# mountaindust/Parasitoids

Measured on AMD Instinct MI355X. Metric: grid-days/sec on 4096^2 fp64 domain, higher is better.
Workload: dtype f64; 1 GPU; C3 synthetic stack: N=4097 (nominal 4096^2), 30 Gaussian day kernels K=2049, reference torus P=5121, FFT size 5184 (fast mode), prob model, one replica stack per GPU; dom_len=4097, ndays=30, P=5121, fft_len=5184, kernels_direct=False, full_column_pipeline=True

## Files before the change

### include/parasitoid_hip.h

```cpp
#ifndef PARASITOID_HIP_H
#define PARASITOID_HIP_H
#include <stdint.h>

#ifdef __cplusplus
extern "C" {
#endif

#define PS_OK 0
#define PS_ERR_NO_DEVICE (-1)
#define PS_ERR_OOM (-2)
#define PS_ERR_BAD_SHAPE (-3)
#define PS_ERR_BAD_ARG (-4)
#define PS_ERR_UNSUPPORTED (-5)
#define PS_ERR_HIP (-6)
#define PS_ERR_HPROB_BOUNDS (-7)
#define PS_ERR_PMF_NEGATIVE (-8)
#define PS_ERR_FLIGHT_PROB (-9)
#define PS_ERR_STATE (-10)
#define PS_ERR_EMPTY (-11)

#define PS_MODE_EXACT 0
#define PS_MODE_FAST 1
#define PS_MODE_FOLD 2
#define PS_MODE_AUTO 3

typedef struct ps_solver ps_solver;
typedef struct ps_model ps_model;

typedef struct ps_day_stats {
  int64_t nnz;
  double sum;
  double delta;
  double padmax;
  int32_t flag;
  int32_t pad_;
} ps_day_stats;

int ps_version(void);
int ps_device_count(void);
const char* ps_last_error(void);
int ps_device_info(int device, char* name, int n, int* cus, int64_t* hbm_bytes);
int ps_row_live_units(int P, int M, int np, int nd, const int32_t* ranges, int32_t* day, int32_t* unit, int cap);
int ps_row_fwd_info(int fft_len, int* np, int* persistent);
int ps_row_fwd_stage_info(int fft_len, int K, int* staged);
int64_t ps_row_fwd_stage_lds(int fft_len, int K);
int64_t ps_row_fwd_stage_bytes(int np, int K);
int ps_row_fwd_stage_slot(int K, int r, int e, int col);
int ps_row_fwd_stage_walk(int K, int64_t rows, int64_t row, int r, int nstaged, int64_t* image);


int ps_solver_create(ps_solver** out, int device, int dom_len, int max_shape, int mode);
int ps_fast_size(int dom_len, int max_shape);
int ps_solver_retarget(ps_solver* s, int max_shape);
int ps_solver_destroy(ps_solver* s);
int ps_solver_info(ps_solver* s, int* dom_len, int* P, int* Pfft, int* H);
int ps_solver_sync(ps_solver* s);
int ps_solver_set_option(ps_solver* s, const char* key, double value);
int ps_solver_get_option(ps_solver* s, const char* key, double* value);
int ps_solver_kernels_direct(ps_solver* s);
int ps_solver_pipeline(ps_solver* s);
int ps_solver_deferred_info(ps_solver* s, int* pending, int64_t* counts);
int ps_solver_auto_info(ps_solver* s, int* first_fold_day, int* fold_fft);
int ps_solver_auto_route(ps_solver* s, int first, int count, int32_t* owner);

int ps_solver_set_state_coo(ps_solver* s, const int32_t* row, const int32_t* col,
                            const double* val, int64_t nnz);

int ps_solver_fftconv2_coo(ps_solver* s, const int32_t* row, const int32_t* col,
                           const double* val, int64_t nnz, int kshape);

int ps_solver_get_cursol(ps_solver* s, double negval, double stat_scale, int renorm,
                         ps_day_stats* stats);

int ps_solver_back_solve(ps_solver* s, int nfilt, const int64_t* off, const int32_t* row,
                         const int32_t* col, const double* val, double negval,
// ... 450 lines not shown
```

### parasitoids_amd/_lib.py

```python
import ctypes as C
import os

import numpy as np

_HERE = os.path.dirname(os.path.abspath(__file__))
LIB_PATH = os.path.join(_HERE, 'libparasitoid_hip.so')

PS_OK = 0
PS_ERR_NO_DEVICE = -1
PS_ERR_OOM = -2
PS_ERR_BAD_SHAPE = -3
PS_ERR_BAD_ARG = -4
PS_ERR_UNSUPPORTED = -5
PS_ERR_HIP = -6
PS_ERR_HPROB_BOUNDS = -7
PS_ERR_PMF_NEGATIVE = -8
PS_ERR_FLIGHT_PROB = -9
PS_ERR_STATE = -10
PS_ERR_EMPTY = -11

MODE_EXACT = 0
MODE_FAST = 1
MODE_FOLD = 2
MODE_AUTO = 3

REC_CHAIN, REC_BACK, REC_STATE, REC_WSUM = 0, 1, 2, 3
REC_NONE = -1


class DayStats(C.Structure):
    _fields_ = [('nnz', C.c_int64), ('sum', C.c_double), ('delta', C.c_double),
                ('padmax', C.c_double), ('flag', C.c_int32), ('pad_', C.c_int32)]


class HipError(RuntimeError):
    def __init__(self, code, msg):
        super().__init__('libparasitoid_hip error %d: %s' % (code, msg))
        self.code = code


_I32P = C.POINTER(C.c_int32)
_I64P = C.POINTER(C.c_int64)
_F64P = C.POINTER(C.c_double)
_VP = C.c_void_p

SIGNATURES = {
    'ps_version': (C.c_int, []),
    'ps_device_count': (C.c_int, []),
    'ps_last_error': (C.c_char_p, []),
    'ps_device_info': (C.c_int, [C.c_int, C.c_char_p, C.c_int, _I32P, _I64P]),
    'ps_row_live_units': (C.c_int, [C.c_int, C.c_int, C.c_int, C.c_int, _I32P, _I32P, _I32P, C.c_int]),
    'ps_row_fwd_info': (C.c_int, [C.c_int, _I32P, _I32P]),
    'ps_row_fwd_stage_info': (C.c_int, [C.c_int, C.c_int, _I32P]),
    'ps_row_fwd_stage_lds': (C.c_int64, [C.c_int, C.c_int]),
    'ps_row_fwd_stage_bytes': (C.c_int64, [C.c_int, C.c_int]),
    'ps_row_fwd_stage_slot': (C.c_int, [C.c_int, C.c_int, C.c_int, C.c_int]),
    'ps_row_fwd_stage_walk': (C.c_int, [C.c_int, C.c_int64, C.c_int64, C.c_int, C.c_int, _I64P]),
    'ps_solver_create': (C.c_int, [C.POINTER(_VP), C.c_int, C.c_int, C.c_int, C.c_int]),
    'ps_solver_destroy': (C.c_int, [_VP]),
    'ps_solver_info': (C.c_int, [_VP, _I32P, _I32P, _I32P, _I32P]),
    'ps_solver_sync': (C.c_int, [_VP]),
    'ps_solver_set_option': (C.c_int, [_VP, C.c_char_p, C.c_double]),
    'ps_solver_get_option': (C.c_int, [_VP, C.c_char_p, _F64P]),
    'ps_solver_set_state_coo': (C.c_int, [_VP, _I32P, _I32P, _F64P, C.c_int64]),
    'ps_solver_fftconv2_coo': (C.c_int, [_VP, _I32P, _I32P, _F64P, C.c_int64, C.c_int]),
    'ps_solver_get_cursol': (C.c_int, [_VP, C.c_double, C.c_double, C.c_int, C.POINTER(DayStats)]),
    'ps_solver_back_solve': (C.c_int, [_VP, C.c_int, _I64P, _I32P, _I32P, _F64P, C.c_double,
                                       C.c_double, C.POINTER(DayStats)]),
    'ps_chain_set_kernels': (C.c_int, [_VP, C.c_int, _I64P, _I32P, _I32P, _I32P, _F64P]),
    'ps_chain_run': (C.c_int, [_VP, C.c_int, C.c_int, C.c_double, C.c_double, C.c_int]),
    'ps_chain_stats': (C.c_int, [_VP, C.c_int, C.c_int, C.POINTER(DayStats)]),
    'ps_chain_run_release': (C.c_int, [_VP, C.c_int, C.c_int, C.c_double, C.c_int, C.c_int, _F64P,
                                       C.POINTER(C.c_int)]),
    'ps_record_stats': (C.c_int, [_VP, C.c_int, C.c_int, C.c_double, C.c_double, C.c_int,
                                  C.POINTER(DayStats)]),
    'ps_solver_retarget': (C.c_int, [_VP, C.c_int]),
    'ps_fast_size': (C.c_int, [C.c_int, C.c_int]),
    'ps_solver_kernels_direct': (C.c_int, [_VP]),
    'ps_solver_pipeline': (C.c_int, [_VP]),
    'ps_solver_deferred_info': (C.c_int, [_VP, _I32P, _I64P]),
    'ps_solver_auto_info': (C.c_int, [_VP, _I32P, _I32P]),
    'ps_solver_auto_route': (C.c_int, [_VP, C.c_int, C.c_int, _I32P]),
    'ps_record_fetch_coo': (C.c_int, [_VP, C.c_int, C.c_int, C.c_double, C.c_double, C.c_double,
                                      C.c_double, _I32P, _I32P, _F64P, C.c_int64, _I64P]),
# ... 377 lines not shown
```

### parasitoids_amd/csrc/fft_colfull_kernels.h

```cpp
#pragma once
#include "fft_rs_kernels.h"

struct ColFullArgs {
  const cplx* src;
  int64_t src_bstride;
  cplx* state;
  int64_t state_bstride;
  cplx* dst;
  int64_t dst_bstride;
  int ld, ncols, mode, store_prod;
  int nd;
  int dst_t;
  int dst_jb, dst_cc, dst_rst;
  int64_t src_dstride, dst_dstride;
  RowLive live;
  const unsigned long long* pred;
  double* pad_energy;
  int pad_row0, ncols_total;
  int col0;
  const cplx* alt_src;
  const unsigned long long* alt_pred;
  RowLive alt_live;
  FftProg prog;
};

inline void colfull_set_layout(ColFullArgs& a, int lay, int L) {
  a.dst_t = lay;
  a.dst_jb = lay == 2 ? 1 - a.ld : 0;
  a.dst_cc = lay == 1 ? L : (lay == 2 ? 2 : 1);
  a.dst_rst = lay == 1 ? 1 : a.ld;
}
#define PS_COLFULL_OFF(a, c, j) ((unsigned)((j) * (a).dst_rst + ((j) & 1) * (a).dst_jb + (c) * (a).dst_cc))

static __global__ void k_pad_quiet(const double* energy, int ncols, double P, double scale, double pad_floor, int* quiet) {
// ... 310 lines not shown
    p = cmul(p, *e);
    *e = p;
  }
  state[col] = p;
}

template <int R1, int R2, int R3>
struct RsDual {
  using S = Rs<R1, R2, R3>;
  static constexpr int L = S::L;
  static constexpr int QA2 = (R2 + 1) / 2, QA3 = (R3 + 1) / 2;
  static constexpr int IA = QA2 * S::T2, IB = QA3 * S::T3;
  static constexpr int JA1 = IA / 16, JA2 = 16 * QA3;
  static constexpr int OFF1 = IA + IA / 16, OFF2 = IB + IB / 16;
  static constexpr int mx(int a, int b) { return a > b ? a : b; }
  static constexpr int MAXEL = mx(mx(IA, L - IA), mx(IB, L - IB));
  static constexpr int XH = (MAXEL + MAXEL / 16 + 32 + 15) & ~15;
  static constexpr size_t fixed_bytes = 2 * (size_t)XH * sizeof(double) + (size_t)L * sizeof(cplx);
  static constexpr long spare = (long)160 * 1024 - (long)fixed_bytes;
  static constexpr int CAP = spare > 0 ? (int)(spare / (64 * (long)sizeof(cplx))) * 64 : 0;
  static constexpr bool ok = S::NTHR <= 384 && CAP >= 512 &&
                             (S::RMAX <= 18 || (S::RMAX == 20 && (R2 * R3 == 20 * 14 || R2 * R3 == 20 * 16)));
  static constexpr size_t bytes = fixed_bytes + (size_t)CAP * sizeof(cplx);
  static_assert(S::T2 % 16 == 0 && S::T3 % 16 == 0, "half-pass offsets assume whole padding groups");
};

template <int R1, int R2, int R3>
__global__ void __launch_bounds__((2 * Rs<R1, R2, R3>::NTHR)) k_colfull_dual(ColFullArgs a) {
  using S = Rs<R1, R2, R3>;
  using D = RsDual<R1, R2, R3>;
  constexpr int L = S::L;
  constexpr int NW = S::NTHR / 64;
  if (pred_skip(a.pred)) return;
  const int b = blockIdx.x, xcd = b & 7, qq = b >> 3;
  const int c = a.col0 + ((((qq >> 3) << 3) + xcd) << 3) + (qq & 7);
  if (c >= a.ncols) return;
  const int role = threadIdx.x / S::NTHR;
  const int j0 = threadIdx.x - role * S::NTHR;
  double* exh = reinterpret_cast<double*>(ps_lds_raw) + role * D::XH;
  cplx* sst = reinterpret_cast<cplx*>(reinterpret_cast<double*>(ps_lds_raw) + 2 * D::XH);
  cplx* stage = sst + L;
  const FftProg& P = a.prog;
  const cplx w2c = tw_lookup(P.tw_lo, P.tw_hi, P.tw_shift, S::tw2(j0));
  const cplx w3c = tw_lookup(P.tw_lo, P.tw_hi, P.tw_shift, j0 < S::T3 ? S::tw3(j0) : 0);
  cplx* st = a.state + (int64_t)blockIdx.y * a.state_bstride + (int64_t)c * L;
  const int nd = a.nd;
  const int lane = j0 & 63, wave = j0 >> 6;

  auto live_of = [&](int day, int& a1, int& b1, int& a2, int& b2) {
    if (!a.live.on) { a1 = 0; b1 = L; a2 = L; b2 = L; return; }
    int lo = 0, hi = 0x3fffffff;
    if (a.live.range) { lo = a.live.range[2 * ((int)blockIdx.y + day)]; hi = a.live.range[2 * ((int)blockIdx.y + day) + 1]; }
    const SrcMap& m = a.live.map;
    a1 = max(0, lo - m.off1); b1 = min(m.n1, hi - m.off1 + 1);
    a2 = m.lo2 + max(0, lo - m.off2); b2 = min(L, m.lo2 + hi - m.off2 + 1);
    if (b1 < a1) b1 = a1;
    if (b2 < a2) b2 = a2;
    if (a2 < b1) a2 = b1;
  };
  auto stage_column = [&](int day) {
    int a1, b1, a2, b2;
    live_of(day, a1, b1, a2, b2);
    const int len1 = b1 - a1, tot = min(len1 + (b2 - a2), D::CAP);
    const cplx* sc = a.src + (int64_t)blockIdx.y * a.src_bstride + (int64_t)day * a.src_dstride + (int64_t)c * L;
    for (int ch = wave; ch * 64 < tot; ch += NW) {
      int e = ch * 64 + lane;
      e = e < tot ? e : tot - 1;
      const int n = e < len1 ? a1 + e : a2 + (e - len1);
      __builtin_amdgcn_global_load_lds(sc + n, (ps_lds_ptr)(stage + ch * 64), 16, 0, 0);
    }
  };

  if (role == 1) {
    stage_column(0);
    PS_WAIT_VM0();
  }
  PS_BAR_LDS();

  for (int slot = 0; slot <= nd; ++slot) {
    const bool act = role == 0 ? slot >= 1 : slot < nd;
    cplx x[S::RMAX];
    int j = j0;
    cplx w2 = w2c, w3 = w3c;
    asm volatile("" : "+v"(j), "+v"(w2.x), "+v"(w2.y), "+v"(w3.x), "+v"(w3.y));
    if (role == 0 && slot == 0) {
#pragma unroll 7
      for (int k = j; k < L; k += S::NTHR) sst[k] = st[k];
    }
    if (act && j < S::T1) {
      if (role == 0) {
#pragma unroll
        for (int q = 0; q < R1; ++q) x[q] = cconj(sst[j + q * S::T1]);
      } else {
        int a1, b1, a2, b2;
        live_of(slot, a1, b1, a2, b2);
        const int len1 = b1 - a1, len2 = b2 - a2;
        if (len1 + len2 <= D::CAP) {
#pragma unroll
          for (int q = 0; q < R1; ++q) {
            const int n = j + q * S::T1;
            const unsigned d1 = (unsigned)(n - a1), d2 = (unsigned)(n - a2);
            const bool in1 = d1 < (unsigned)len1, in2 = d2 < (unsigned)len2;
            const cplx v = stage[in1 ? d1 : (in2 ? len1 + d2 : 0u)];
            x[q] = (in1 || in2) ? v : make_double2(0.0, 0.0);
          }
        } else {
          const cplx* sc = a.src + (int64_t)blockIdx.y * a.src_bstride + (int64_t)slot * a.src_dstride + (int64_t)c * L;
#pragma unroll
          for (int q = 0; q < R1; ++q) {
            const int n = j + q * S::T1;
            x[q] = make_double2(0.0, 0.0);
            int e = -1;
            if (n >= a1 && n < b1) e = n - a1;
            else if (n >= a2 && n < b2) e = len1 + (n - a2);
            if (e >= 0) x[q] = e < D::CAP ? stage[e] : sc[n];
          }
        }
      }
      bfly<R1, PS_FWD>(x);
    }
#pragma unroll
    for (int part = 0; part < 2; ++part) {
      double keep[D::QA2];
#pragma unroll
      for (int h = 0; h < 2; ++h) {
        if (act && j < S::T1 && (j < D::JA1) == (h == 0)) {
          if (part) rs_put<R1, 1>(exh, S::x1_w(j) - h * D::OFF1, 1, x);
          else rs_put<R1, 0>(exh, S::x1_w(j) - h * D::OFF1, 1, x);
        }
        PS_BAR_LDS();
        if (part == 0 && h == 0 && role == 1 && slot + 1 < nd) stage_column(slot + 1);
        if (act && j < S::T2) {
          if (h == 0) {
#pragma unroll
            for (int q = 0; q < D::QA2; ++q) keep[q] = exh[S::x_r(j) + q * S::X1_RS];
          } else {
#pragma unroll
            for (int q = D::QA2; q < R2; ++q) {
              const double v = exh[S::x_r(j) + q * S::X1_RS - D::OFF1];
              if (part) x[q].y = v;
              else x[q].x = v;
            }
#pragma unroll
            for (int q = 0; q < D::QA2; ++q) {
              if (part) x[q].y = keep[q];
              else x[q].x = keep[q];
            }
          }
        }
        if (!(part == 1 && h == 1)) PS_BAR_LDS();
      }
    }
    asm volatile("" : "+v"(w2.x), "+v"(w2.y));
    if (act && j < S::T2) rs_stage<R2, PS_FWD>(x, w2, true);
    PS_BAR_LDS();
#pragma unroll
    for (int part = 0; part < 2; ++part) {
      double keep[D::QA3];
#pragma unroll
      for (int h = 0; h < 2; ++h) {
        if (act && j < S::T2 && (j < D::JA2) == (h == 0)) {
          if (part) rs_put<R2, 1>(exh, S::x2_w(j) - h * D::OFF2, 17, x);
          else rs_put<R2, 0>(exh, S::x2_w(j) - h * D::OFF2, 17, x);
        }
        PS_BAR_LDS();
        if (act && j < S::T3) {
          if (h == 0) {
#pragma unroll
            for (int q = 0; q < D::QA3; ++q) keep[q] = exh[S::x_r(j) + q * S::X2_RS];
          } else {
#pragma unroll
            for (int q = D::QA3; q < R3; ++q) {
              const double v = exh[S::x_r(j) + q * S::X2_RS - D::OFF2];
              if (part) x[q].y = v;
              else x[q].x = v;
            }
#pragma unroll
            for (int q = 0; q < D::QA3; ++q) {
              if (part) x[q].y = keep[q];
              else x[q].x = keep[q];
            }
          }
        }
        if (!(part == 1 && h == 1)) PS_BAR_LDS();
      }
    }
    asm volatile("" : "+v"(w3.x), "+v"(w3.y));
    if (act && j < S::T3) rs_stage<R3, PS_FWD>(x, w3, true);
    if (act && j < S::T3) {
      if (role == 0) {
        const int64_t rst = a.dst_rst;
        cplx* d = a.dst + (int64_t)blockIdx.y * a.dst_bstride + (int64_t)(slot - 1) * a.dst_dstride + PS_COLFULL_OFF(a, c, j);
#pragma unroll
        for (int q = 0; q < R3; ++q) d[(int64_t)(q * S::T3) * rst] = cconj(x[q]);
      } else {
#pragma unroll
        for (int q = 0; q < R3; ++q) {
          const cplx p = cmul(sst[j + q * S::T3], x[q]);
          sst[j + q * S::T3] = p;
        }
      }
    }
    if (role == 1 && slot == nd && a.store_prod) {
      for (int k = j; k < L; k += S::NTHR) st[k] = sst[k];
    }
    if (role == 0 && a.pad_energy) {
      double pe = 0.0;
      if (act && j < S::T3) {
        const int qlo = a.pad_row0 / S::T3;
#pragma unroll
        for (int q = 0; q < R3; ++q) {
          if (q < qlo) continue;
          if (q > qlo || j + q * S::T3 >= a.pad_row0) pe += x[q].x * x[q].x + x[q].y * x[q].y;
        }
      }
      pe = ps_wave_sum(pe);
      if (lane == 63) exh[D::XH - 8 + wave] = pe;
    }
    if (role == 1) PS_WAIT_VM0();
    PS_BAR_LDS();
    if (role == 0 && a.pad_energy && slot >= 1 && j0 == 0) {
      double e = 0.0;
      for (int w = 0; w < NW; ++w) e += exh[D::XH - 8 + w];
      a.pad_energy[((int64_t)blockIdx.y + (slot - 1)) * a.ncols_total + c] = e;
    }
  }
}
```

### parasitoids_amd/csrc/ps_coldual.hip

```cpp
#include "fft_colfull_kernels.h"
#include "rs_cfg.h"
#include "rs_launch.h"

template <int A, int B>
struct DualCfg {
  using D = RsDual<16, A, B>;
  using C = RsCfg<A, B>;
  static constexpr bool on = D::ok && C::CHAIN && C::LDSC > (size_t)80 * 1024;
};

bool rs_dual_ok(int r2, int r3) {
#define X(A, B) \
  if (r2 == A && r3 == B) return DualCfg<A, B>::on;
  PS_RS_SIZES(X)
#undef X
  return false;
}

int rs_coldual_set_attrs() {
#define X(A, B)                                                                                         \
  if constexpr (DualCfg<A, B>::on) {                                                                    \
    using DD = RsDual<16, A, B>;                                                                        \
    auto kern = k_colfull_dual<16, A, B>;                                                               \
    if (hipFuncSetAttribute((const void*)kern, hipFuncAttributeMaxDynamicSharedMemorySize, (int)DD::bytes) != hipSuccess) \
      return -1;                                                                                        \
  }
  PS_RS_SIZES(X)
#undef X
  return 0;
}

int rs_launch_coldual(int r2, int r3, const ColFullArgs& a, int lines8, int batch, hipStream_t st) {
  const dim3 grid((unsigned)(lines8 * 64), batch);
#define X(A, B)                                                                                         \
  if (r2 == A && r3 == B) {                                                                             \
    if constexpr (DualCfg<A, B>::on) {                                                                  \
      using DD = RsDual<16, A, B>;                                                                      \
      auto kern = k_colfull_dual<16, A, B>;                                                             \
      hipLaunchKernelGGL(kern, grid, dim3(2 * DD::S::NTHR), DD::bytes, st, a);                          \
      return 1;                                                                                         \
    }                                                                                                   \
    return 0;                                                                                           \
  }
  PS_RS_SIZES(X)
#undef X
  return 0;
}
```

### parasitoids_amd/csrc/ps_config.h

```cpp
#pragma once
#include <cstdlib>
#include <cstring>

#define PS_OPTION_TABLE(X)                                                                          \
                                               \
  X("PS_NO_RS", no_rs, 0, FLAG, C)                                                                  \
  X("PS_NO_RS_FWD", no_rs_fwd, 0, FLAG, C)                                                          \
  X("PS_NO_BIG_RADIX", no_big_radix, 0, FLAG, C)                                                    \
  X("PS_NO_TPIPE", no_tpipe, 0, FLAG, C)                                                            \
  X("PS_NO_FOLD_TPIPE", no_fold_tpipe, 0, FLAG, C)                                                  \
  X("PS_COL_SINGLE_MAX", col_single_max, 1200, INT, C)                                              \
  X("PS_COL_L1", col_l1, 0, INT, C)                                                                 \
  X("PS_CHUNK_DAYS", chunk_days, 0, INT, C)                                                         \
  X("PS_FAST_SIZE", fast_size, 0, INT, C)                                                           \
  X("PS_RS_AREA", rs_area, 0.0, NUM, C)                                                             \
                                                                                 \
  X("PS_COL_WSH", col_wsh, -1, INT, R)                                                              \
  X("PS_COL_THREADS", col_threads, 256, INT, R)                                                     \
  X("PS_FUSED_WSH", fused_wsh, -1, INT, R)                                                          \
  X("PS_FUSED_THREADS", fused_threads, 0, INT, R)                                                   \
  X("PS_FUSED_G", fused_g, 2, INT, R)                                                               \
  X("PS_MULTI_WSH", multi_wsh, -1, INT, R)                                                          \
  X("PS_DUAL_WSH", dual_wsh, -1, INT, R)                                                            \
  X("PS_FUSED_DAYS", fused_days, 8, INT, R)                                                         \
  X("PS_DIRECT_DAYS", direct_days, 4, INT, R)                                                       \
  X("PS_DIRECT_MAX_TERMS", direct_max_terms, 8, INT, R)                                             \
  X("PS_TPIPE_DAYS", tpipe_days, 32, INT, R)                                                        \
  X("PS_DUAL_MIN_DAYS", dual_min_days, 6, INT, R)                                                   \
                                                   \
  X("PS_TINV", tinv, 0, INT, R)                                                                     \
  X("PS_RSP", rsp, -1, INT, R)                                                                      \
  X("PS_ROW2", row2, -1, INT, R)                                                                    \
  X("PS_TPIPE", tpipe, -1, INT, R)                                                                  \
  X("PS_NO_PAIR_ROWS", no_pair_rows, 0, FLAG, R)                                                    \
  X("PS_TPIPE_SPLIT", tpipe_split, 0, INT, R)                                                       \
  X("PS_NO_CONJ", no_conj, 0, FLAG, R)                                                              \
  X("PS_NO_DUAL", no_dual, 0, FLAG, R)                                                              \
  X("PS_NO_DIRECT", no_direct, 0, FLAG, R)                                                          \
  X("PS_NO_ROW_BATCH", no_row_batch, 0, FLAG, R)                                                    \
  X("PS_NO_PAD_QUIET", no_pad_quiet, 0, FLAG, R)                                                    \
  X("PS_NO_TAIL_SPLIT", no_tail_split, 0, FLAG, R)                                                  \
  X("PS_NO_FWD_PERSIST", no_fwd_persist, 0, FLAG, R)                                                \
  X("PS_NO_FWD_SOLO", no_fwd_solo, 0, FLAG, R)                                                      \
  X("PS_FWD_STAGE", fwd_stage, 0, FLAG, R)                                                          \
  X("PS_NO_DEFER_REFFT", no_defer_refft, 0, FLAG, R)                                                \
  X("PS_NO_FILTER_CACHE", no_filter_cache, 0, FLAG, R)                                              \
  X("PS_NO_FOLD_FUSE", no_fold_fuse, 0, FLAG, R)                                                    \
  X("PS_NO_FOLD_ALT", no_fold_alt, 0, FLAG, R)                                                      \
  X("PS_NO_FOLD_ROWS", no_fold_rows, 0, FLAG, R)                                                    \
                                                                                 \
  X("PS_NO_SPECULATION", no_speculation, 0, FLAG, R)                                                \
  X("PS_SPEC_DEPTH", spec_depth, 2, INT, R)                                                         \
  X("PS_NO_FLAG_HISTORY", no_flag_history, 0, FLAG, R)                                              \
  X("PS_NO_WINDOW_HINT", no_window_hint, 0, FLAG, R)                                                \
  X("PS_NO_DEFER_CHECK", no_defer_check, 0, FLAG, R)                                                \
  X("PS_FIRST_WINDOW", first_window, -1, INT, R)                                                    \
  X("PS_KT_SPLIT", kt_split, -1, INT, R)                                                            \
  X("PS_NO_LAZY_KT", no_lazy_kt, 0, FLAG, R)                                                        \
  X("PS_NO_WIDE", no_wide, 0, FLAG, R)                                                              \
  X("PS_NO_ROUTE_HISTORY", no_route_history, 0, FLAG, R)                                            \
  X("PS_WIDE_MIN_N", wide_min_n, 1500, INT, R)                                                      \
  X("PS_AUTO_WINDOW", auto_window, 4, INT, R)                                                       \
                                                                  \
  X("PS_PM_SEG", pm_seg, 8, INT, R)                                                                 \
  X("PS_PM_SYNC", pm_sync, 0, FLAG, R)                                                              \
  X("PS_PM_NO_UNROLL", pm_no_unroll, 0, FLAG, R)

struct ps_config {
#define PS_CFG_FIELD_FLAG int
#define PS_CFG_FIELD_INT int
#define PS_CFG_FIELD_NUM double
#define X(key, field, dflt, kind, when) PS_CFG_FIELD_##kind field = dflt;
  PS_OPTION_TABLE(X)
#undef X
// ... 43 lines not shown
```

### parasitoids_amd/csrc/ps_solver.hip

```cpp
#include <deque>

#include "chain_kernels.h"
#include "fft_kernels.h"
#include "fft_colfull_kernels.h"
#include "rs_launch.h"
#include "row_fwd_stage.h"
#include "ps_common.h"
#include "ps_config.h"

thread_local std::string ps_tls_error;

extern "C" const char* ps_last_error(void) { return ps_tls_error.c_str(); }
extern "C" int ps_version(void) { return 100; }
extern "C" int ps_row_live_units(int P, int M, int np, int nd, const int32_t* ranges, int32_t* day, int32_t* unit, int cap) {
  if (!ranges && nd > 0) return -1;
  if (cap > 0 && (!day || !unit)) return -1;
  return rs_row_live_units(P, M, np, nd, ranges, day, unit, cap);
}
extern "C" int ps_row_fwd_info(int fft_len, int* np, int* persistent) {
  int r2 = 0, r3 = 0, n = 0, p = 0;
  if (!rs_lookup(fft_len, &r2, &r3) || !rs_row_fwd_info(r2, r3, &n, &p)) return -1;
  if (np) *np = n;
  if (persistent) *persistent = p;
  return 0;
}

extern "C" int ps_row_fwd_stage_info(int fft_len, int K, int* staged) {
  int r2 = 0, r3 = 0, n = 0, p = 0;
  if (K < 1 || !rs_lookup(fft_len, &r2, &r3) || !rs_row_fwd_info(r2, r3, &n, &p)) return -1;
  if (staged) *staged = p && rs_row_fwd_staged(r2, r3, K) ? 1 : 0;
  return 0;
}
extern "C" int64_t ps_row_fwd_stage_bytes(int np, int K) { return np < 1 || K < 1 ? -1 : (int64_t)fstage_bytes(np, K); }
extern "C" int64_t ps_row_fwd_stage_lds(int fft_len, int K) {
  int r2 = 0, r3 = 0;
  if (K < 1 || !rs_lookup(fft_len, &r2, &r3)) return -1;
  return (int64_t)rs_row_fwd_stage_lds(r2, r3, K);
}
extern "C" int ps_row_fwd_stage_slot(int K, int r, int e, int col) {
  return K < 1 || r < 0 || (e != 0 && e != 1) || col < 0 || col >= K ? -1 : fstage_slot(K, r, e, col);
}
extern "C" int ps_row_fwd_stage_walk(int K, int64_t rows, int64_t row, int r, int nstaged, int64_t* image) {
  if (K < 1 || !(K & 1) || rows < 1 || row < 0 || row >= rows || r < 0 || r >= nstaged || !image) return -1;
  const int e = (int)((row * K) & 1);
  const int64_t base = row * K - e, room = rows * K - base;
  for (int ch = 0; ch < fstage_chunks(K); ++ch)
    for (int lane = 0; lane < 64; ++lane) {
      const int w = fstage_word(K, e, room, ch, lane);
      const int d = fstage_slot(K, r, 0, 0) + ch * 128 + 2 * lane;
      if (w >= 0) { image[d] = base + 2 * (int64_t)w; image[d + 1] = base + 2 * (int64_t)w + 1; }
// ... 451 lines not shown
  a.rowsum = s->rowsum.p + (int64_t)stat_slot * s->N;
  a.rowcnt = s->rowcnt.p + (int64_t)stat_slot * s->N;
  a.padmax = s->padmax.p + stat_slot;
  a.pad_floor = s->pad_floor;
  a.stat_bstride = s->N;
  if (full_field) {
    a.N = s->Pf;
    a.rec_bstride = (int64_t)s->Pf * s->Pf;
    a.rowsum = s->fold_rowsum.p; a.rowcnt = s->fold_rowcnt.p; a.padmax = s->fold_padmax.p;
    a.stat_bstride = s->Pf;
  }
  const int npairs = (s->Pf + 1) / 2;
  dim3 grid((npairs + a.rp - 1) / a.rp, batch);
  const int thr = row_threads(a.prog.L, s->row_big);
  const size_t lds = ((size_t)a.rp * row_pitch(a.prog) + a.prog.n_lo + a.prog.n_hi + a.prog.n_gen) * sizeof(cplx) +
                     4 * (thr / 64) * sizeof(double);
  if (lds > (size_t)kMaxLds) return ps_fail(PS_ERR_UNSUPPORTED, "row pass needs %zu B LDS", lds);
  ProfScope prof(s, !recs_multi ? PS_PROF_ROW_INV : batch == 2 ? PS_PROF_ROW_INV2 : batch == 4 ? PS_PROF_ROW_INV4
                                : batch == 8 ? PS_PROF_ROW_INV8 : batch == 1 ? PS_PROF_ROW_INV : PS_PROF_ROW_INVN,
                 recs_multi ? batch : 1);
  if (s->rs_r2 != 0) {
    if (!rs_launch_row_inv(s->rs_r2, s->rs_r3, a, npairs, batch, s->stream))
      return ps_fail(PS_ERR_STATE, "no register-resident row kernel for 16 x %d x %d", s->rs_r2, s->rs_r3);
  } else if (s->row_plan.generic)
    hipLaunchKernelGGL((k_row_inv<true, false>), grid, dim3(thr), lds, s->stream, a);
  else if (s->row_big)
    hipLaunchKernelGGL((k_row_inv<false, true>), grid, dim3(thr), lds, s->stream, a);
  else
    hipLaunchKernelGGL((k_row_inv<false, false>), grid, dim3(thr), lds, s->stream, a);
  PS_HIP(hipGetLastError());
  return PS_OK;
}

static bool colfull_dual(const ps_solver* s, int nd) {
  const int dual_min = s->cfg.dual_min_days;
  return dual_min > 0 && nd >= dual_min && rs_dual_ok(s->rs_r2, s->rs_r3);
}

static SrcMap map_plain(int n, int P);
struct ColAlt { const cplx* src; const unsigned long long* pred; RowLive live; };

static int launch_colfull(ps_solver* s, int mode, const cplx* src, cplx* state, int store_prod, cplx* dst, int batch,
                          RowLive live, const unsigned long long* pred, int nd = 1, double* pad_energy = nullptr,
                          int col0 = 0, int ncols = -1, int64_t state_bstride = -1, bool timed = true,
                          const ColAlt* alt = nullptr) {
  ColFullArgs a;
  a.pad_energy = nullptr;
  a.alt_src = nullptr; a.alt_pred = nullptr; a.alt_live = RowLive{0, {0, 0, 0, 0}, nullptr};
  if (alt) {
    if (!(mode == 0 && nd == 1 && batch == 1 && !pred) || s->refft_pending)
      return ps_fail(PS_ERR_STATE, "full-column pass: an alternative state source needs a plain single-day pass");
    a.alt_src = alt->src; a.alt_pred = alt->pred; a.alt_live = alt->live;
  }
  if (s->refft_pending) {
    if (!(mode == 0 && nd == 1 && batch == 1 && !pred && state == s->Ahat.p))
      return ps_fail(PS_ERR_STATE, "full-column pass: a flagged day's re-transform is still pending");
    a.alt_src = s->Trow.p; a.alt_pred = s->refft_pending;
    a.alt_live = RowLive{1, map_plain(s->N, s->Pf), nullptr};
  }
  a.pad_row0 = 2 * ((s->N + 1) / 2);
  a.ncols_total = s->H;
  a.col0 = col0;
  const int64_t spec = (int64_t)s->Pf * s->ld;
  a.src = src; a.src_bstride = spec;
  a.state = state; a.state_bstride = state_bstride >= 0 ? state_bstride : spec;
  a.dst = dst; a.dst_bstride = spec;
  a.ld = s->ld; a.ncols = ncols >= 0 ? ncols : s->H; a.mode = mode; a.store_prod = store_prod;
  a.nd = nd; a.src_dstride = spec; a.dst_dstride = spec;
  colfull_set_layout(a, s->tinv ? 1 : inter_layout(s), s->Pf);
  a.live = live;
  a.pred = pred;
  a.prog = s->row_plan.prog;
  const int groups = (a.ncols - col0 + 7) / 8;
  const int lines8 = (groups + 7) / 8;
  if (mode == 2) a.pad_energy = pad_energy;
  const bool prof_was = s->prof_on;
  if (!timed) s->prof_on = false;
  ProfScope prof(s, pred ? PS_PROF_REFFT
                          : (mode == 1 ? PS_PROF_COL_FWD_A
                                       : (nd == 2 ? PS_PROF_COL_INV_A2 : nd == 4 ? PS_PROF_COL_INV_A4
                                          : nd == 8 ? PS_PROF_COL_INV_A8 : nd == 1 ? PS_PROF_COL_INV_A : PS_PROF_COL_INV_AN)),
                 nd);
  s->prof_on = prof_was;
  if (mode == 0 && !pred && store_prod && colfull_dual(s, nd)) {
    a.pad_energy = pad_energy;
    if (!rs_launch_coldual(s->rs_r2, s->rs_r3, a, lines8, batch, s->stream))
      return ps_fail(PS_ERR_STATE, "two-role full-column pass: size 16 x %d x %d is not served", s->rs_r2, s->rs_r3);
    PS_HIP(hipGetLastError());
    return PS_OK;
  }
  if (!rs_launch_colfull(s->rs_r2, s->rs_r3, a, lines8, batch, s->stream))
    return ps_fail(PS_ERR_UNSUPPORTED, "full-column pass: size 16 x %d x %d cannot run this (chained days need the state column in LDS)",
                   s->rs_r2, s->rs_r3);
  PS_HIP(hipGetLastError());
  return PS_OK;
}

static bool colfull_chains(const ps_solver* s) {
  RsInfo info;
  return rs_info(s->rs_r2, s->rs_r3, &info) && info.chain;
}

static int fwd2d(ps_solver* s, const double* src, int64_t src_bstride, int src_ld, SrcMap rmap,
                 SrcMap cmap, cplx* out, int batch, const unsigned long long* pred, const int* rowrange = nullptr) {
  PS_TRY(launch_row_fwd(s, src, src_bstride, src_ld, rmap, cmap, s->T1.p, batch, pred, 1, rowrange));
  if (s->tpipe) return launch_colfull(s, 1, s->T1.p, out, 0, nullptr, batch, RowLive{1, rmap, rowrange}, pred);
  if (s->fwd_passes.size() == 1) {
    PS_TRY(launch_col<PS_FWD>(s, s->fwd_passes[0], s->T1.p, nullptr, nullptr, out, batch, 0, pred, RowLive{1, rmap, rowrange}));
  } else {
    PS_TRY(launch_col<PS_FWD>(s, s->fwd_passes[0], s->T1.p, nullptr, nullptr, s->T2.p, batch, 0, pred, RowLive{1, rmap, rowrange}));
    PS_TRY(launch_col<PS_FWD>(s, s->fwd_passes[1], s->T2.p, nullptr, nullptr, out, batch, 0, pred));
  }
  return PS_OK;
}

static int inv2d(ps_solver* s, const cplx* A, const cplx* B, cplx* prod, double* rec,
                 int stat_slot, double negval, double stat_scale) {
  if (s->tpipe) {
    if (B || prod) return ps_fail(PS_ERR_STATE, "inv2d: product form is not used by the full-column pipeline");
// ... 178 lines not shown
    const int split2 = s->cfg.tpipe_split;
    if (split2 && store_prod) {
      PS_TRY(launch_colfull(s, 3, kt, state, 1, nullptr, 1, live, nullptr));
      PS_TRY(launch_colfull(s, 2, nullptr, state, 0, s->T1.p, 1, RowLive{0, {0, 0, 0, 0}, nullptr}, nullptr));
    } else {
      PS_TRY(launch_colfull(s, 0, kt, state, store_prod, s->T1.p, 1, live, nullptr));
    }
    return launch_row_inv(s, s->T1.p, rec, stat_slot, 1, negval, stat_scale);
  }
  int done = 0;
  if (s->kt_direct && store_prod) PS_TRY(launch_col_fused_multi(s, kt, 1, state, s->T1.p, rowrange, &done));
  if (!done) PS_TRY(launch_col_fused(s, kt, state, store_prod, s->T1.p, rowrange));
  if (!s->split) return launch_row_inv(s, s->T1.p, rec, stat_slot, 1, negval, stat_scale);
  PS_TRY(launch_col<PS_INV>(s, s->inv_passes[1], s->T1.p, nullptr, nullptr, s->T2.p, 1, 0, nullptr));
  return launch_row_inv(s, s->T2.p, rec, stat_slot, 1, negval, stat_scale);
}

static int conv_inv_multi(ps_solver* s, const cplx* kt, int nd, cplx* state, double* const* recs, int d0,
                          double negval, double stat_scale, const int* rowrange, int* done) {
  const size_t spec = (size_t)s->Pf * s->ld;
  PS_TRY(s->T1.ensure(spec * nd));
  if (s->tpipe) {
    *done = 0;
    if (!colfull_chains(s)) return PS_OK;
    RowLive live = s->kt_live;
    live.range = rowrange;
    const bool batched_rows = row_inv_persistent(s) && !s->tinv && nd <= PS_MAX_GROUP_DAYS && !s->cfg.no_row_batch;
    const bool quiet = batched_rows && colfull_dual(s, nd) && s->N + 1 < s->Pf && !s->cfg.no_pad_quiet;
    if (quiet) {
      PS_TRY(s->pad_energy.ensure((size_t)nd * s->H));
      PS_TRY(s->pad_quiet.ensure(PS_MAX_GROUP_DAYS));
    }
    int hmain = s->H;
    if (!s->ncu) {
      int v = 0;
      if (hipDeviceGetAttribute(&v, hipDeviceAttributeMultiprocessorCount, s->device) == hipSuccess) s->ncu = v;
    }
    if (colfull_dual(s, nd) && s->ncu > 0 && s->H > s->ncu && !s->tinv && !s->cfg.no_tail_split) {
      const int rem = s->H % s->ncu;
      if (rem > 0 && rem * 3 <= s->ncu) hmain = s->H - rem;
    }
    PS_TRY(launch_colfull(s, 0, kt, state, 1, s->T1.p, 1, live, nullptr, nd, quiet ? s->pad_energy.p : nullptr, 0, hmain));
    if (hmain < s->H) {
      const int rem = s->H - hmain;
      PS_TRY(s->tail_hat.ensure((size_t)nd * rem * s->Pf));
      cplx* th = s->tail_hat.p - (int64_t)hmain * s->Pf;
      {
        ProfScope prof(s, PS_PROF_COL_TAIL, nd);
        PS_TRY(launch_colfull(s, 1, kt, th, 0, nullptr, nd, live, nullptr, 1, nullptr, hmain, s->H, (int64_t)rem * s->Pf, false));
        hipLaunchKernelGGL(k_prefix_cols, dim3((s->Pf + 255) / 256, rem), dim3(256), 0, s->stream,
                           state + (int64_t)hmain * s->Pf, s->tail_hat.p, s->Pf, rem, nd);
        PS_HIP(hipGetLastError());
        PS_TRY(launch_colfull(s, 2, nullptr, th, 0, s->T1.p, nd, RowLive{0, {0, 0, 0, 0}, nullptr}, nullptr, 1,
                              quiet ? s->pad_energy.p : nullptr, hmain, s->H, (int64_t)rem * s->Pf, false));
      }
    }
    if (quiet) {
      hipLaunchKernelGGL(k_pad_quiet, dim3(nd), dim3(256), 0, s->stream, s->pad_energy.p, s->H, (double)s->Pf,
                         1.0 / ((double)s->Pf * (double)s->Pf), s->pad_floor, s->pad_quiet.p);
      PS_HIP(hipGetLastError());
    }
    if (batched_rows) {
      PS_TRY(launch_row_inv(s, s->T1.p, nullptr, d0, nd, negval, stat_scale, false, recs, quiet ? s->pad_quiet.p : nullptr));
    } else {
      for (int i = 0; i < nd; ++i)
        PS_TRY(launch_row_inv(s, s->T1.p + i * spec, recs[i], d0 + i, 1, negval, stat_scale));
    }
    *done = 1;
    return PS_OK;
  }
// ... 1949 lines not shown
```

### parasitoids_amd/csrc/rs_launch.h

```cpp
#pragma once
#include <hip/hip_runtime.h>
#include "fft_kernels.h"

struct ColFullArgs;

struct RsInfo {
  int np, nthr;
  size_t lds_rows, lds_col1, lds_colc;
  bool chain;
  bool rsp;
};
bool rs_lookup(int L, int* r2, int* r3);
int rs_next_size(int n);
bool rs_info(int r2, int r3, RsInfo* out);
int rs_rows_set_attrs();
int rs_colfull_set_attrs();
int rs_launch_row_fwd(int r2, int r3, const RowFwdArgs& a, int npairs, int batch, hipStream_t st);
int rs_launch_row_inv(int r2, int r3, const RowInvArgs& a, int npairs, int batch, hipStream_t st);
bool rs_row_fwd_info(int r2, int r3, int* np, int* persistent);
int rs_launch_row_fwd_live(int r2, int r3, const RowFwdArgs& a, const int* hranges, int batch, hipStream_t st,
                           bool stage, bool solo);
size_t rs_row_fwd_stage_lds(int r2, int r3, int src_ld);
bool rs_row_fwd_staged(int r2, int r3, int src_ld);
int rs_row_live_units(int P, int M, int np, int nd, const int* ranges, int* day, int* unit, int cap);
int rs_launch_colfull(int r2, int r3, const ColFullArgs& a, int lines8, int batch, hipStream_t st);
struct RowFoldArgs;
int rs_launch_row_fold(int r2, int r3, const RowFoldArgs& a, int units, hipStream_t st);
bool rs_colfull_alt_ok(int r2, int r3);
bool rs_dual_ok(int r2, int r3);
int rs_coldual_set_attrs();
int rs_launch_coldual(int r2, int r3, const ColFullArgs& a, int lines8, int batch, hipStream_t st);
```

Baseline: 4475 grid-days/s.

## Add persistent-workgroup schedule to two-role column FFT pass

Adds an optional persistent mode for the dual-role full-column kernel. Each workgroup walks several columns in a strided schedule, and role B overlaps the next column's staging and state load with the current compute, also handling the store-back of the previous column. By default the grid equals the padded column count, so each block still covers one column, while the loop, the LDS state load via global_load_lds and the deferred store-back are new. The persistent grid sized to the CU count is enabled only through PS_COL_PERSIST.

```diff
diff --git a/include/parasitoid_hip.h b/include/parasitoid_hip.h
--- a/include/parasitoid_hip.h
+++ b/include/parasitoid_hip.h
@@ -41,6 +41,8 @@
 const char* ps_last_error(void);
 int ps_device_info(int device, char* name, int n, int* cus, int64_t* hbm_bytes);
 int ps_row_live_units(int P, int M, int np, int nd, const int32_t* ranges, int32_t* day, int32_t* unit, int cap);
+int ps_coldual_schedule(int nwg, int col0, int ncols, int nd, int b, int32_t* col_b, int32_t* day_b,
+                        int32_t* col_a, int32_t* day_a, int32_t* sw, int cap);
 int ps_row_fwd_info(int fft_len, int* np, int* persistent);
 int ps_row_fwd_stage_info(int fft_len, int K, int* staged);
 int64_t ps_row_fwd_stage_lds(int fft_len, int K);
diff --git a/parasitoids_amd/_lib.py b/parasitoids_amd/_lib.py
--- a/parasitoids_amd/_lib.py
+++ b/parasitoids_amd/_lib.py
@@ -50,6 +50,7 @@
     'ps_last_error': (C.c_char_p, []),
     'ps_device_info': (C.c_int, [C.c_int, C.c_char_p, C.c_int, _I32P, _I64P]),
     'ps_row_live_units': (C.c_int, [C.c_int, C.c_int, C.c_int, C.c_int, _I32P, _I32P, _I32P, C.c_int]),
+    'ps_coldual_schedule': (C.c_int, [C.c_int, C.c_int, C.c_int, C.c_int, C.c_int, _I32P, _I32P, _I32P, _I32P, _I32P, C.c_int]),
     'ps_row_fwd_info': (C.c_int, [C.c_int, _I32P, _I32P]),
     'ps_row_fwd_stage_info': (C.c_int, [C.c_int, C.c_int, _I32P]),
     'ps_row_fwd_stage_lds': (C.c_int64, [C.c_int, C.c_int]),
diff --git a/parasitoids_amd/csrc/coldual_sched.h b/parasitoids_amd/csrc/coldual_sched.h
--- /dev/null
+++ b/parasitoids_amd/csrc/coldual_sched.h
@@ -0,0 +1,57 @@
+#pragma once
+#include "fft_core.h"
+
+PS_HD int coldual_column(int col0, int vb) {
+  const int xcd = vb & 7, qq = vb >> 3;
+  return col0 + ((((qq >> 3) << 3) + xcd) << 3) + (qq & 7);
+}
+
+PS_HD int coldual_count(int b, int nwg, int col0, int ncols) {
+  const int c = coldual_column(col0, b);
+  return c >= ncols ? 0 : (ncols - 1 - c) / nwg + 1;
+}
+
+struct ColDualSlot {
+  int g, total;
+  int cb, dayb;
+  int ca, daya;
+};
+PS_HD ColDualSlot coldual_begin(int b, int nwg, int col0, int ncols, int nd) {
+  return ColDualSlot{0, coldual_count(b, nwg, col0, ncols) * nd, coldual_column(col0, b), 0, -1, -1};
+}
+PS_HD bool coldual_act_a(const ColDualSlot& s) { return s.g >= 1; }
+PS_HD bool coldual_act_b(const ColDualSlot& s) { return s.g < s.total; }
+PS_HD bool coldual_switch(const ColDualSlot& s) { return s.g > 0 && s.g < s.total && s.dayb == 0; }
+PS_HD bool coldual_has_next(const ColDualSlot& s) { return s.g + 1 < s.total; }
+PS_HD int coldual_next_day(const ColDualSlot& s, int nd) { return s.dayb + 1 == nd ? 0 : s.dayb + 1; }
+PS_HD int coldual_next_col(const ColDualSlot& s, int nd, int nwg) { return s.dayb + 1 == nd ? s.cb + nwg : s.cb; }
+PS_HD void coldual_advance(ColDualSlot& s, int nd, int nwg) {
+  s.ca = s.cb;
+  s.daya = s.dayb;
+  s.cb = coldual_next_col(s, nd, nwg);
+  s.dayb = coldual_next_day(s, nd);
+  ++s.g;
+}
+
+inline int coldual_schedule(int nwg, int col0, int ncols, int nd, int b, int32_t* col_b, int32_t* day_b,
+                            int32_t* col_a, int32_t* day_a, int32_t* sw, int cap) {
+  if (nwg < 64 || nwg % 64 || col0 < 0 || ncols < col0 || nd < 1 || b < 0 || b >= nwg || cap < 0) return -1;
+  if (cap > 0 && (!col_b || !day_b || !col_a || !day_a || !sw)) return -1;
+  if ((int64_t)ncols + nwg > 0x7fffffff || (int64_t)(ncols - col0) * nd > 0x3fffffff) return -1;
+  ColDualSlot s = coldual_begin(b, nwg, col0, ncols, nd);
+  if (s.total == 0) return 0;
+  for (; s.g <= s.total && s.g < cap; coldual_advance(s, nd, nwg)) {
+    const bool aa = coldual_act_a(s), ab = coldual_act_b(s);
+    col_b[s.g] = ab ? s.cb : -1;
+    day_b[s.g] = ab ? s.dayb : -1;
+    col_a[s.g] = aa ? s.ca : -1;
+    day_a[s.g] = aa ? s.daya : -1;
+    sw[s.g] = coldual_switch(s) ? 1 : 0;
+  }
+  return s.total + 1;
+}
+
+PS_HD int coldual_grid(int n, int ncu, bool persist) {
+  const int percol = ((n + 63) / 64) * 64, cus = (ncu / 64) * 64;
+  return persist && cus >= 64 && cus < percol ? cus : percol;
+}
diff --git a/parasitoids_amd/csrc/fft_colfull_kernels.h b/parasitoids_amd/csrc/fft_colfull_kernels.h
--- a/parasitoids_amd/csrc/fft_colfull_kernels.h
+++ b/parasitoids_amd/csrc/fft_colfull_kernels.h
@@ -1,5 +1,6 @@
 #pragma once
 #include "fft_rs_kernels.h"
+#include "coldual_sched.h"
 
 struct ColFullArgs {
   const cplx* src;
@@ -376,9 +377,10 @@
   constexpr int L = S::L;
   constexpr int NW = S::NTHR / 64;
   if (pred_skip(a.pred)) return;
-  const int b = blockIdx.x, xcd = b & 7, qq = b >> 3;
-  const int c = a.col0 + ((((qq >> 3) << 3) + xcd) << 3) + (qq & 7);
-  if (c >= a.ncols) return;
+  const int nd = a.nd;
+  const int nwg = gridDim.x;
+  ColDualSlot sl = coldual_begin(blockIdx.x, nwg, a.col0, a.ncols, nd);
+  if (sl.total == 0) return;
   const int role = threadIdx.x / S::NTHR;
   const int j0 = threadIdx.x - role * S::NTHR;
   double* exh = reinterpret_cast<double*>(ps_lds_raw) + role * D::XH;
@@ -387,8 +389,7 @@
   const FftProg& P = a.prog;
   const cplx w2c = tw_lookup(P.tw_lo, P.tw_hi, P.tw_shift, S::tw2(j0));
   const cplx w3c = tw_lookup(P.tw_lo, P.tw_hi, P.tw_shift, j0 < S::T3 ? S::tw3(j0) : 0);
-  cplx* st = a.state + (int64_t)blockIdx.y * a.state_bstride + (int64_t)c * L;
-  const int nd = a.nd;
+  cplx* stb = a.state + (int64_t)blockIdx.y * a.state_bstride;
   const int lane = j0 & 63, wave = j0 >> 6;
 
   auto live_of = [&](int day, int& a1, int& b1, int& a2, int& b2) {
@@ -402,7 +403,7 @@
     if (b2 < a2) b2 = a2;
     if (a2 < b1) a2 = b1;
   };
-  auto stage_column = [&](int day) {
+  auto stage_column = [&](int c, int day) {
     int a1, b1, a2, b2;
     live_of(day, a1, b1, a2, b2);
     const int len1 = b1 - a1, tot = min(len1 + (b2 - a2), D::CAP);
@@ -414,22 +415,33 @@
       __builtin_amdgcn_global_load_lds(sc + n, (ps_lds_ptr)(stage + ch * 64), 16, 0, 0);
     }
   };
+  auto load_state = [&](int c, int jj) {
+    constexpr int NCH = L / 64, REM = L % 64;
+    const cplx* sc = stb + (int64_t)c * L;
+    const int ln = jj & 63, wv = __builtin_amdgcn_readfirstlane(jj >> 6);
+    for (int ch = wv; ch < NCH; ch += NW)
+      __builtin_amdgcn_global_load_lds(sc + ch * 64 + ln, (ps_lds_ptr)(sst + ch * 64), 16, 0, 0);
+    if (REM > 0 && wv == NCH % NW && ln < REM)
+      __builtin_amdgcn_global_load_lds(sc + NCH * 64 + ln, (ps_lds_ptr)(sst + NCH * 64), 16, 0, 0);
+  };
 
   if (role == 1) {
-    stage_column(0);
+    stage_column(sl.cb, 0);
+    load_state(sl.cb, j0);
     PS_WAIT_VM0();
   }
   PS_BAR_LDS();
 
-  for (int slot = 0; slot <= nd; ++slot) {
-    const bool act = role == 0 ? slot >= 1 : slot < nd;
+  for (; sl.g <= sl.total; coldual_advance(sl, nd, nwg)) {
+    const bool act = role == 0 ? coldual_act_a(sl) : coldual_act_b(sl);
+    const bool sw = coldual_switch(sl);
     cplx x[S::RMAX];
     int j = j0;
     cplx w2 = w2c, w3 = w3c;
     asm volatile("" : "+v"(j), "+v"(w2.x), "+v"(w2.y), "+v"(w3.x), "+v"(w3.y));
-    if (role == 0 && slot == 0) {
-#pragma unroll 7
-      for (int k = j; k < L; k += S::NTHR) sst[k] = st[k];
+    if (role == 1 && sl.g > 0 && sl.dayb == 0 && a.store_prod) {
+      cplx* st = stb + (int64_t)(sl.cb - nwg) * L;
+      for (int k = j; k < L; k += S::NTHR) st[k] = sst[k];
     }
     if (act && j < S::T1) {
       if (role == 0) {
@@ -437,7 +449,7 @@
         for (int q = 0; q < R1; ++q) x[q] = cconj(sst[j + q * S::T1]);
       } else {
         int a1, b1, a2, b2;
-        live_of(slot, a1, b1, a2, b2);
+        live_of(sl.dayb, a1, b1, a2, b2);
         const int len1 = b1 - a1, len2 = b2 - a2;
         if (len1 + len2 <= D::CAP) {
 #pragma unroll
@@ -449,7 +461,7 @@
             x[q] = (in1 || in2) ? v : make_double2(0.0, 0.0);
           }
         } else {
-          const cplx* sc = a.src + (int64_t)blockIdx.y * a.src_bstride + (int64_t)slot * a.src_dstride + (int64_t)c * L;
+          const cplx* sc = a.src + (int64_t)blockIdx.y * a.src_bstride + (int64_t)sl.dayb * a.src_dstride + (int64_t)sl.cb * L;
 #pragma unroll
           for (int q = 0; q < R1; ++q) {
             const int n = j + q * S::T1;
@@ -473,7 +485,10 @@
           else rs_put<R1, 0>(exh, S::x1_w(j) - h * D::OFF1, 1, x);
         }
         PS_BAR_LDS();
-        if (part == 0 && h == 0 && role == 1 && slot + 1 < nd) stage_column(slot + 1);
+        if (part == 0 && h == 0 && role == 1) {
+          if (coldual_has_next(sl)) stage_column(coldual_next_col(sl, nd, nwg), coldual_next_day(sl, nd));
+          if (sw) load_state(sl.cb, j);
+        }
         if (act && j < S::T2) {
           if (h == 0) {
 #pragma unroll
@@ -507,6 +522,7 @@
           if (part) rs_put<R2, 1>(exh, S::x2_w(j) - h * D::OFF2, 17, x);
           else rs_put<R2, 0>(exh, S::x2_w(j) - h * D::OFF2, 17, x);
         }
+        if (part == 1 && h == 1 && role == 1 && sw) PS_WAIT_VM0();
         PS_BAR_LDS();
         if (act && j < S::T3) {
           if (h == 0) {
@@ -534,7 +550,7 @@
     if (act && j < S::T3) {
       if (role == 0) {
         const int64_t rst = a.dst_rst;
-        cplx* d = a.dst + (int64_t)blockIdx.y * a.dst_bstride + (int64_t)(slot - 1) * a.dst_dstride + PS_COLFULL_OFF(a, c, j);
+        cplx* d = a.dst + (int64_t)blockIdx.y * a.dst_bstride + (int64_t)sl.daya * a.dst_dstride + PS_COLFULL_OFF(a, sl.ca, j);
 #pragma unroll
         for (int q = 0; q < R3; ++q) d[(int64_t)(q * S::T3) * rst] = cconj(x[q]);
       } else {
@@ -544,9 +560,6 @@
           sst[j + q * S::T3] = p;
         }
       }
-    }
-    if (role == 1 && slot == nd && a.store_prod) {
-      for (int k = j; k < L; k += S::NTHR) st[k] = sst[k];
     }
     if (role == 0 && a.pad_energy) {
       double pe = 0.0;
@@ -563,10 +576,10 @@
     }
     if (role == 1) PS_WAIT_VM0();
     PS_BAR_LDS();
-    if (role == 0 && a.pad_energy && slot >= 1 && j0 == 0) {
+    if (role == 0 && a.pad_energy && act && j0 == 0) {
       double e = 0.0;
       for (int w = 0; w < NW; ++w) e += exh[D::XH - 8 + w];
-      a.pad_energy[((int64_t)blockIdx.y + (slot - 1)) * a.ncols_total + c] = e;
+      a.pad_energy[((int64_t)blockIdx.y + sl.daya) * a.ncols_total + sl.ca] = e;
     }
   }
 }
diff --git a/parasitoids_amd/csrc/ps_coldual.hip b/parasitoids_amd/csrc/ps_coldual.hip
--- a/parasitoids_amd/csrc/ps_coldual.hip
+++ b/parasitoids_amd/csrc/ps_coldual.hip
@@ -30,8 +30,9 @@
   return 0;
 }
 
-int rs_launch_coldual(int r2, int r3, const ColFullArgs& a, int lines8, int batch, hipStream_t st) {
-  const dim3 grid((unsigned)(lines8 * 64), batch);
+int rs_launch_coldual(int r2, int r3, const ColFullArgs& a, int nwg, int batch, hipStream_t st) {
+  if (nwg < 64 || nwg % 64) return 0;
+  const dim3 grid((unsigned)nwg, batch);
 #define X(A, B)                                                                                         \
   if (r2 == A && r3 == B) {                                                                             \
     if constexpr (DualCfg<A, B>::on) {                                                                  \
diff --git a/parasitoids_amd/csrc/ps_config.h b/parasitoids_amd/csrc/ps_config.h
--- a/parasitoids_amd/csrc/ps_config.h
+++ b/parasitoids_amd/csrc/ps_config.h
@@ -40,6 +40,7 @@
   X("PS_NO_ROW_BATCH", no_row_batch, 0, FLAG, R)                                                    \
   X("PS_NO_PAD_QUIET", no_pad_quiet, 0, FLAG, R)                                                    \
   X("PS_NO_TAIL_SPLIT", no_tail_split, 0, FLAG, R)                                                  \
+  X("PS_COL_PERSIST", col_persist, 0, FLAG, R)                                                      \
   X("PS_NO_FWD_PERSIST", no_fwd_persist, 0, FLAG, R)                                                \
   X("PS_NO_FWD_SOLO", no_fwd_solo, 0, FLAG, R)                                                      \
   X("PS_FWD_STAGE", fwd_stage, 0, FLAG, R)                                                          \
diff --git a/parasitoids_amd/csrc/ps_solver.hip b/parasitoids_amd/csrc/ps_solver.hip
--- a/parasitoids_amd/csrc/ps_solver.hip
+++ b/parasitoids_amd/csrc/ps_solver.hip
@@ -5,6 +5,7 @@
 #include "fft_colfull_kernels.h"
 #include "rs_launch.h"
 #include "row_fwd_stage.h"
+#include "coldual_sched.h"
 #include "ps_common.h"
 #include "ps_config.h"
 
@@ -16,6 +17,10 @@
   if (!ranges && nd > 0) return -1;
   if (cap > 0 && (!day || !unit)) return -1;
   return rs_row_live_units(P, M, np, nd, ranges, day, unit, cap);
+}
+extern "C" int ps_coldual_schedule(int nwg, int col0, int ncols, int nd, int b, int32_t* col_b, int32_t* day_b,
+                                   int32_t* col_a, int32_t* day_a, int32_t* sw, int cap) {
+  return coldual_schedule(nwg, col0, ncols, nd, b, col_b, day_b, col_a, day_a, sw, cap);
 }
 extern "C" int ps_row_fwd_info(int fft_len, int* np, int* persistent) {
   int r2 = 0, r3 = 0, n = 0, p = 0;
@@ -533,6 +538,14 @@
   return PS_OK;
 }
 
+static int solver_ncu(ps_solver* s) {
+  if (!s->ncu) {
+    int v = 0;
+    if (hipDeviceGetAttribute(&v, hipDeviceAttributeMultiprocessorCount, s->device) == hipSuccess) s->ncu = v;
+  }
+  return s->ncu;
+}
+
 static bool colfull_dual(const ps_solver* s, int nd) {
   const int dual_min = s->cfg.dual_min_days;
   return dual_min > 0 && nd >= dual_min && rs_dual_ok(s->rs_r2, s->rs_r3);
@@ -585,7 +598,8 @@
   s->prof_on = prof_was;
   if (mode == 0 && !pred && store_prod && colfull_dual(s, nd)) {
     a.pad_energy = pad_energy;
-    if (!rs_launch_coldual(s->rs_r2, s->rs_r3, a, lines8, batch, s->stream))
+    const int nwg = coldual_grid(a.ncols - col0, solver_ncu(s), s->cfg.col_persist != 0);
+    if (!rs_launch_coldual(s->rs_r2, s->rs_r3, a, nwg, batch, s->stream))
       return ps_fail(PS_ERR_STATE, "two-role full-column pass: size 16 x %d x %d is not served", s->rs_r2, s->rs_r3);
     PS_HIP(hipGetLastError());
     return PS_OK;
@@ -830,10 +844,7 @@
       PS_TRY(s->pad_quiet.ensure(PS_MAX_GROUP_DAYS));
     }
     int hmain = s->H;
-    if (!s->ncu) {
-      int v = 0;
-      if (hipDeviceGetAttribute(&v, hipDeviceAttributeMultiprocessorCount, s->device) == hipSuccess) s->ncu = v;
-    }
+    solver_ncu(s);
     if (colfull_dual(s, nd) && s->ncu > 0 && s->H > s->ncu && !s->tinv && !s->cfg.no_tail_split) {
       const int rem = s->H % s->ncu;
       if (rem > 0 && rem * 3 <= s->ncu) hmain = s->H - rem;
diff --git a/parasitoids_amd/csrc/rs_launch.h b/parasitoids_amd/csrc/rs_launch.h
--- a/parasitoids_amd/csrc/rs_launch.h
+++ b/parasitoids_amd/csrc/rs_launch.h
@@ -29,4 +29,4 @@
 bool rs_colfull_alt_ok(int r2, int r3);
 bool rs_dual_ok(int r2, int r3);
 int rs_coldual_set_attrs();
-int rs_launch_coldual(int r2, int r3, const ColFullArgs& a, int lines8, int batch, hipStream_t st);
+int rs_launch_coldual(int r2, int r3, const ColFullArgs& a, int nwg, int batch, hipStream_t st);
```

Result: no change. 4473 grid-days/s (-0.0%).
